# tsunrise/r1cs-spartan

Hardware: AMD Instinct MI355X
Metric: R1CS constraints proved/sec at 2^20 (higher is better)
Workload: dtype bls12-381 Fr/Fq Montgomery (u32 limbs)

## Files before the change

r1cs-spartan_amd/csrc/curve29.hpp:

```cpp
#pragma once
#include "curve_dev.hpp"
#include "ff29.hpp"

namespace spx {

template <class S>
struct R29;
template <>
struct R29<Fq> {
    using T = F29;
    static DEV void unpack(F29& r, const Fq& s) { f29_unpack(r, s.v); }
    static DEV void pack(Fq& s, const F29& r) { f29_pack(s.v, r); }
};
template <>
struct R29<Fq2> {
    using T = F2_29;
    static DEV void unpack(F2_29& r, const Fq2& s) {
        f29_unpack(r.c0, s.c0.v);
        f29_unpack(r.c1, s.c1.v);
    }
    static DEV void pack(Fq2& s, const F2_29& r) {
        f29_pack(s.c0.v, r.c0);
        f29_pack(s.c1.v, r.c1);
    }
// ... 80 lines not shown
template <class F>
DEV void x29_dbl(X29<F>& p) {
    using O = Ops29<F>;
    if (x29_is_inf(p)) return;
    F U, V, W, S, X2, M, t, s2;
    O::add(U, p.y, p.y);
    O::sqr(V, U);
    O::mul(W, U, V);
    O::mul(S, p.x, V);
    O::sqr(X2, p.x);
    O::add(M, X2, X2);
    O::add(M, M, X2);
    O::sqr(t, M);
    O::add(s2, S, S);
    F x3;
    O::template sub<4>(x3, t, s2);
    O::template reduce<8>(x3);
    O::template sub<2>(t, S, x3);
    if constexpr (O::kFusedSum) {
        O::zero(s2);
        O::template sub<2>(s2, s2, W);
        O::mul_sum(p.y, M, t, s2, p.y);
    } else {
        O::mul(t, M, t);
        O::mul(s2, W, p.y);
        O::template sub<2>(p.y, t, s2);
        O::template reduce<4>(p.y);
    }
    p.x = x3;
    O::mul(p.zz, V, p.zz);
    O::mul(p.zzz, W, p.zzz);
}

template <class F>
DEV void x29_madd(X29<F>& p, const F& ax, const F& ay_in, bool neg) {
    using O = Ops29<F>;
    F ay = ay_in;
    if (neg) {
        F z;
        O::zero(z);
        O::template sub<2>(ay, z, ay_in);
    }
    if (x29_is_inf(p)) {
        p.x = ax;
        p.y = ay;
        O::one(p.zz);
        O::one(p.zzz);
        return;
    }
    F U2, S2, P, R;
    O::mul_x2(U2, ax, p.zz, S2, ay, p.zzz);
    O::template sub<8>(P, U2, p.x);
    O::template sub<4>(R, S2, p.y);
    if (O::template zero_lt<16>(P)) {
        if (O::template zero_lt<8>(R))
            x29_from_aff_dbl(p, ax, ay);
        else
            x29_set_inf(p);
        return;
    }
    F PP, PPP, Q, t, w;
    O::template sqr_x2<16, 8>(PP, P, t, R);
    O::mul_x2(PPP, P, PP, Q, p.x, PP);
    O::template sub<2>(w, t, PPP);
    O::add(t, Q, Q);
    O::template sub<4>(w, w, t);
    O::template sub<8>(t, Q, w);
    O::zero(S2);
    O::template sub<4>(S2, S2, p.y);
    O::mul_sum(p.y, t, R, S2, PPP);
    p.x = w;
    O::mul_x2(p.zz, p.zz, PP, p.zzz, p.zzz, PPP);
}

template <class F>
DEV void x29_add(X29<F>& p, const X29<F>& q) {
    using O = Ops29<F>;
    if (x29_is_inf(q)) return;
    if (x29_is_inf(p)) {
        p = q;
        return;
    }
    F U1, U2, S1, S2, P, R;
    O::mul(U1, p.x, q.zz);
    O::mul(U2, q.x, p.zz);
    O::mul(S1, p.y, q.zzz);
    O::mul(S2, q.y, p.zzz);
    O::template sub<2>(P, U2, U1);
    O::template sub<2>(R, S2, S1);
    if (O::template zero_lt<4>(P)) {
        if (O::template zero_lt<4>(R))
            x29_dbl(p);
        else
            x29_set_inf(p);
        return;
    }
    F PP, PPP, Q, t, w;
    O::sqr(PP, P);
    O::mul(PPP, P, PP);
    O::mul(Q, U1, PP);
    O::sqr(t, R);
    O::template sub<2>(w, t, PPP);
    O::add(t, Q, Q);
    O::template sub<4>(w, w, t);
    O::template reduce<8>(w);
// ... 36 lines not shown
```

r1cs-spartan_amd/csrc/msm_common.hip:

```cpp
#include "msm_common.hpp"

#include <algorithm>
#include <cmath>
#include <cstring>
#include <cstdlib>

namespace spx {

__device__ __constant__ constexpr uint32_t kFqR2[12] = {0x1c341746u, 0xf4df1f34u, 0x09d104f1u, 0x0a76e6a6u,
                                                       0x4c95b6d5u, 0x8de5476cu, 0x939d83c0u, 0x67eb88a9u,
                                                       0xb519952du, 0x9a793e85u, 0x92cae3aau, 0x11988fe5u};

struct Digits {
    uint32_t s[8];
    uint32_t carry = 0;
    DEV int32_t next(uint32_t c) {
        const uint32_t full = 1u << c, half = full >> 1;
        uint32_t v = (s[0] & (full - 1)) + carry;
#pragma unroll
        for (int k = 0; k < 7; ++k) s[k] = (s[k] >> c) | (s[k + 1] << (32 - c));
        s[7] >>= c;
        carry = v > half;
        return carry ? (int32_t)v - (int32_t)full : (int32_t)v;
    }
// ... 46 lines not shown
#pragma unroll
    for (int k = 0; k < 8; ++k) d.s[k] = sc.v[k];
    if (I.c == 16 && I.W == 16) {
#pragma unroll
        for (uint32_t w = 0; w < 16; ++w) {
            const int32_t dg = d.at16(w);
            k16.key[w] = digit_key(I, dg);
            k16.ref[w] = digit_ref(I, w, j, dg);
        }
        return true;
    }
    const uint32_t flip = I.c == kMsmWideBits ? d.fold_half() : 0u;
    if (I.c == kMsmWideBits && I.W == kMsmWideWindows) {
#pragma unroll
        for (uint32_t w = 0; w < kMsmWideWindows; ++w) {
            const int32_t dg = d.at17(w);
            k16.key[w] = digit_key(I, dg);
            k16.ref[w] = digit_ref(I, w, j, dg) ^ flip;
        }
        k16.key[15] = ~0u;
        k16.ref[15] = 0u;
        return true;
    }
    for (uint32_t w = 0; w < I.W; ++w) {
        const int32_t dg = d.next(I.c);
        const uint32_t key = digit_key(I, dg);
        if (key != ~0u) f(key, digit_ref(I, w, j, dg) ^ flip);
    }
    return false;
}

static constexpr int kTileThreads = 1024;
static constexpr int kRowThreads = 1024;
static constexpr int kScanThreads = 256;
static constexpr int kBinThreads = 1024;
static constexpr uint32_t kMaxBins = 2048;
static constexpr uint32_t kStagePairs = (uint32_t)kTileThreads * 16;
static constexpr uint32_t kBinStage = 36864;
static constexpr int kMaxLev = 8;
static_assert(((uint64_t)kMaxBins << 8) == kMsmMaxBuckets, "kMsmMaxBuckets (kernels.hpp): kMaxBins bins of 2^8 buckets");
typedef __attribute__((address_space(1))) unsigned int gu32;

struct SortGeom {
    uint32_t nb, sb, nbin;
    uint32_t spt, ntile;
    uint32_t sub;
    uint64_t tot_sc;
};

template <int NT>
DEV uint32_t block_excl_scan(uint32_t v, uint32_t& agg, uint32_t* sh) {
    const int lane = threadIdx.x & 63, w = threadIdx.x >> 6;
    uint32_t x = v;
#pragma unroll
    for (int d = 1; d < 64; d <<= 1) {
        const uint32_t y = __shfl_up(x, d, 64);
        if (lane >= d) x += y;
    }
    if (lane == 63) sh[w] = x;
    __syncthreads();
    uint32_t pre = 0;
    agg = 0;
#pragma unroll
    for (int k = 0; k < NT / 64; ++k) {
        const uint32_t t = sh[k];
        pre += k < w ? t : 0u;
// ... 188 lines not shown
            const uint32_t q = lds_inc(pos, key >> g.sb);
            sref[q] = ref;
            sfine[q] = (uint8_t)(key & fmask);
        };
        if (scalar_keys(insts, prefix, nact, scalars, gi, kk, put)) {
            uint32_t q[16];
#pragma unroll
            for (int w = 0; w < 16; ++w) {
                q[w] = 0u;
                if (kk.key[w] != ~0u) q[w] = lds_inc(pos, kk.key[w] >> g.sb);
            }
#pragma unroll
            for (int w = 0; w < 16; ++w)
                if (kk.key[w] != ~0u) {
                    sref[q[w]] = kk.ref[w];
                    sfine[q[w]] = (uint8_t)(kk.key[w] & fmask);
                }
        }
    }
}

template <int NT, uint32_t STAGE>
struct BinLds {
    uint32_t out[STAGE ? STAGE : 1];
    uint32_t h[256], sh[NT / 64];
};
struct LevPtrs {
    uint32_t* p[kMaxLev + 1];
};
template <int NT, uint32_t STAGE>
__global__ __launch_bounds__(NT) void k_sort_bins(SortGeom g, const uint32_t* __restrict__ binbase,
                                                            uint32_t* __restrict__ st, const uint32_t* __restrict__ sref,
                                                            const uint8_t* __restrict__ sfine, uint32_t* __restrict__ offs,
                                                            uint32_t* __restrict__ refs, uint32_t seg1, int nlev, LevPtrs lev,
                                                            uint32_t* __restrict__ binsum, uint32_t* __restrict__ binpfx,
                                                            uint32_t* __restrict__ ticket, uint32_t* __restrict__ hot,
                                                            uint32_t hot_cap) {
    __shared__ BinLds<NT, STAGE> L;
    __shared__ bool last;
    const uint32_t bin = blockIdx.x, f = threadIdx.x;
    const uint32_t b0 = bin << g.sb, nbk = min(1u << g.sb, g.nb - b0);
    const bool over = (st[0] & kMsmOverflow) != 0;
    const uint32_t base = binbase[bin], n = over ? 0u : binbase[bin + 1] - base;
    const uint32_t a0 = base & ~3u, head = base - a0, nq = n ? (head + n + 3) / 4 : 0u;
    if (f < 256) L.h[f] = 0;
    __syncthreads();
    for (uint32_t q = f; q < nq; q += NT) {
        const uint32_t w4 = *(const uint32_t*)(sfine + a0 + 4 * q);
#pragma unroll
        for (uint32_t e = 0; e < 4; ++e)
            if (4 * q + e - head < n) lds_inc(L.h, (w4 >> (8 * e)) & 0xFFu);
    }
    __syncthreads();
    const uint32_t c = f < nbk ? L.h[f] : 0u;
    uint32_t agg;
    const uint32_t lo = block_excl_scan<NT>(c, agg, L.sh);
    const uint32_t o = base + lo;
    if (f < nbk) offs[b0 + f] = over ? 0u : o;
    uint32_t v = c ? (o + c - 1) / seg1 - o / seg1 + 1 : 0u;
    for (int l = 0; l <= nlev; ++l) {
        if (l) v = (v + kSeg - 1) / kSeg;
        const uint32_t e = block_excl_scan<NT>(v, agg, L.sh);
        if (f < nbk) lev.p[l][b0 + f] = e;
        if (f == 0) st_agent(binsum + (size_t)l * (g.nbin + 1) + bin, agg);
    }
    if (v > kSeg) {
        const uint32_t i = atomicAdd(&st[kMsmStHot], 1u);
        if (i < hot_cap) hot[i] = b0 + f;
    }
    const bool staged = n <= STAGE;
    if (f < 256) L.h[f] = staged ? lo : o;
    __syncthreads();
    for (uint32_t q = f; q < nq; q += NT) {
        const uint32_t w4 = *(const uint32_t*)(sfine + a0 + 4 * q);
        const uint4 r4 = *(const uint4*)(sref + a0 + 4 * q);
        const uint32_t rr[4] = {r4.x, r4.y, r4.z, r4.w};
#pragma unroll
        for (uint32_t e = 0; e < 4; ++e)
            if (4 * q + e - head < n) {
                const uint32_t slot = lds_inc(L.h, (w4 >> (8 * e)) & 0xFFu);
                if (staged)
                    L.out[slot] = rr[e];
                else
                    refs[slot] = rr[e];
            }
    }
    if (staged) {
        __syncthreads();
        for (uint32_t i = f; i < n; i += NT) refs[base + i] = L.out[i];
    }
    if (!handoff_last(ticket, g.nbin, &last)) return;
    for (int l = 0; l <= nlev; ++l) {
        uint32_t carry = 0;
        const uint32_t* src = binsum + (size_t)l * (g.nbin + 1);
        uint32_t* dst = binpfx + (size_t)l * (g.nbin + 1);
        for (uint32_t b = 0; b < g.nbin; b += NT) {
            const uint32_t i = b + f;
            const uint32_t x = i < g.nbin ? ld_agent(src + i) : 0u;
            const uint32_t e = block_excl_scan<NT>(x, agg, L.sh);
            if (i < g.nbin) dst[i] = carry + e;
            carry += agg;
        }
        if (f == 0) dst[g.nbin] = carry;
    }
    if (f == 0) *ticket = 0u;
}

__global__ __launch_bounds__(kScanThreads) void k_sort_final(SortGeom g, int nlev, LevPtrs lev, const uint32_t* __restrict__ binpfx) {
    const uint64_t t = blockIdx.x * (uint64_t)kScanThreads + threadIdx.x;
    const uint32_t l = (uint32_t)(t / (g.nb + 1)), b = (uint32_t)(t % (g.nb + 1));
    if ((int)l > nlev) return;
    const uint32_t* pf = binpfx + (size_t)l * (g.nbin + 1);
    lev.p[l][b] = b < g.nb ? lev.p[l][b] + pf[b >> g.sb] : pf[g.nbin];
}

uint32_t seg1_len(bool) { return kSeg1Default; }

uint32_t seg1_fit(uint32_t seg1, uint64_t refs, int waves_per_simd, int lanes_per_elem) {
    static const int cus = [] {
        int dev = 0, n = 0;
        if (hipGetDevice(&dev) != hipSuccess || hipDeviceGetAttribute(&n, hipDeviceAttributeMultiprocessorCount, dev) != hipSuccess)
            n = 0;
        return n;
    }();
    if (cus <= 0 || refs == 0) return seg1;
    const uint64_t slots = (uint64_t)cus * 4 * waves_per_simd * 64 / lanes_per_elem;
    const uint64_t nthr = (refs + seg1 - 1) / seg1;
    const uint64_t rounds = (nthr + slots - 1) / slots;
    if (rounds > 16) return seg1;
    const uint64_t fit = (refs + rounds * slots - 1) / (rounds * slots);
    return (uint32_t)std::min<uint64_t>(seg1, std::max<uint64_t>(fit, std::min<uint32_t>(seg1, 8)));
}
// ... 12 lines not shown
}
void msm_ws_set_hot(MsmWorkspace* ws, bool on) {
    if (ws) ws->hot_on = on;
}
bool msm_hot_default() {
    static const bool v = [] {
        const char* e = getenv("SPX_MSM_HOT");
        return !(e && atoi(e) == 0 && *e);
    }();
    return v;
}
uint32_t msm_hot_cap(uint64_t tot_refs, uint32_t seg1, int nlev) {
    uint64_t per = 1;
    for (int l = 0; l <= nlev; ++l) per *= kSeg;
    const uint64_t cap = tot_refs / ((per - 1) * std::max<uint32_t>(seg1, 1)) + 1;
    if (cap < tot_refs / (per * std::max<uint32_t>(seg1, 1)) + 1) throw std::runtime_error("MSM: hot-bucket list capacity");
    return (uint32_t)std::min<uint64_t>(cap, 0xffffffffu);
}

static double msm_cap_env() {
    const char* e = getenv("SPX_MSM_CAP_SCALE");
    const double v = e ? atof(e) : 1.0;
    return v > 0 ? v : 1.0;
}

MsmPlan msm_plan(const MsmInst* ih, int ninst, const MsmShard& sh, double cap_scale) {
    MsmPlan o;
    const int G = std::max(1, sh.world);
    int g = 0;
    while ((1 << g) < G) ++g;
    if ((1 << g) != G || sh.rank < 0 || sh.rank >= G) throw std::runtime_error("MSM shard: bad rank / world");
    o.compact = G > 1 && !sh.dense;
    uint64_t tot_refs = 0;
    double split_refs = 0, whole_refs = 0;
    int nsplit = 0;
    for (int i = 0; i < ninst; ++i) {
        MsmInst I = ih[i];
        if (!I.size) continue;
        if (I.c < 3 || I.c > 24) throw std::runtime_error("MSM window bits out of range");
        if (I.W < msm_windows(I.c)) throw std::runtime_error("MSM: too few windows for the window bits");
        const uint32_t lbf = I.c - 1;
        if (G > 1 && (int)lbf - g >= 2) {
            I.lb = lbf - g;
            I.lg = (uint32_t)g;
            I.sel = (uint32_t)sh.rank;
            split_refs += (double)I.size * I.W / G;
            ++nsplit;
        } else if (i % G == sh.rank) {
            I.lb = lbf;
            I.lg = 0;
            I.sel = 0;
            whole_refs += (double)I.size * I.W;
        } else {
            continue;
        }
        I.out = (uint32_t)i;
        I.bucket_off = o.nb;
        I.ref_off = (uint32_t)tot_refs;
        o.nb += 1u << I.lb;
        o.prefix.push_back(o.tot_sc);
        o.tot_sc += I.size;
        tot_refs += (uint64_t)I.size * I.W;
        o.mu_max = std::max(o.mu_max, (double)I.size * I.W / (double)(1u << lbf));
        o.any_split |= I.lg != 0;
        o.insts.push_back(I);
    }
    const int nact = (int)o.insts.size();
    o.prefix.push_back(o.tot_sc);
    if (tot_refs >= 0xffffffffull) throw std::runtime_error("MSM batch too large");
    if (o.compact) {
        const double cap = whole_refs + (split_refs + 8.0 * std::sqrt(split_refs) + 2048.0 * nsplit) * cap_scale * msm_cap_env();
        tot_refs = std::min<uint64_t>(tot_refs, (uint64_t)std::ceil(cap));
    }
    o.tot_refs = tot_refs;
    o.node_off.resize(nact);
    o.cnt.resize(nact);
    uint32_t tot_nodes = 0;
    for (int i = 0; i < nact; ++i) {
        o.node_off[i] = tot_nodes;
        const int lg = (int)o.insts[i].lb - (int)std::min<uint32_t>(kTreeChunkLog, o.insts[i].lb - 1);
        o.cnt[i] = 1u << lg;
        tot_nodes += o.cnt[i];
        o.levels = std::max(o.levels, lg);
    }
    o.wp.assign((size_t)(o.levels + 1) * (nact + 1), 0);
    o.cin.assign((size_t)(o.levels + 1) * nact, 0);
    uint32_t maxc = 1;
    for (int i = 0; i < nact; ++i) maxc = std::max(maxc, o.cnt[i]);
    o.top_from = o.levels + 1;
    for (int lv = 0; lv <= o.levels; ++lv) {
        uint64_t acc = 0;
        for (int i = 0; i < nact; ++i) {
            uint32_t nin = lv == 0 ? (o.cnt[i] * 2) : std::max(1u, o.cnt[i] >> (lv - 1));
            uint32_t nout = lv == 0 ? o.cnt[i] : std::max(1u, o.cnt[i] >> lv);
            o.cin[(size_t)lv * nact + i] = nin;
            o.wp[(size_t)lv * (nact + 1) + i] = acc;
            acc += nout;
        }
        o.wp[(size_t)lv * (nact + 1) + nact] = acc;
        if (lv >= 1 && o.top_from > o.levels && std::max(1u, maxc >> (lv - 1)) <= kTopNodes) o.top_from = lv;
    }
    return o;
}

void msm_upload_plan(MsmWorkspace* ws, MsmPlan& p, hipStream_t s) {
    const int nact = (int)p.insts.size();
    auto al = [](size_t x) { return (x + 15) & ~(size_t)15; };
// ... 38 lines not shown
        while (sb > 0 && (double)(1u << sb) * std::max(p.mu_max, 1.0) > 0.8 * kBinStage) --sb;
    else
        sb = std::min(8, std::max(0, lnb - 9));
    while (sb < 8 && ((uint64_t)p.nb + (1u << sb) - 1) >> sb > kMaxBins) ++sb;
    g.sb = (uint32_t)sb;
    g.nbin = (p.nb + (1u << g.sb) - 1) >> g.sb;
    if (g.nbin > kMaxBins) throw std::runtime_error("MSM batch: too many buckets for the sort");
    const int threads = staged ? kTileThreads : kDirectThreads, tiles_log = staged ? 8 : 9;
    const uint64_t tile_sc = (uint64_t)threads << tiles_log;
    g.spt = (uint32_t)std::min<uint64_t>(64, std::max<uint64_t>(1, (p.tot_sc + tile_sc - 1) / tile_sc));
    const uint64_t ts = (uint64_t)threads * g.spt;
    const uint64_t nt = (p.tot_sc + ts - 1) / ts;
    if (nt > 0x7fffffffull / kSub) throw std::runtime_error("MSM batch: too many tiles");
    g.ntile = (uint32_t)std::max<uint64_t>(1, nt);
    g.sub = staged ? kSub : 1;
    return g;
}

MsmSorted msm_sort(MsmWorkspace* ws, const MsmPlan& p, const Fr* scalars, void* out_dev, size_t out_bytes, hipStream_t s,
                   uint32_t seg1, int nlev) {
    if (nlev > kMaxLev) throw std::runtime_error("MSM: too many partial levels");
    if (out_bytes % 4) throw std::runtime_error("MSM: output bytes not a multiple of 4");
    MsmSorted o;
    bool staged = false;
    const SortGeom g = sort_geom(p, staged);
    const uint32_t nb = p.nb;
    const uint64_t cap = std::max<uint64_t>(p.tot_refs, 1);
    uint32_t* st = (uint32_t*)((uint8_t*)out_dev + out_bytes - 16);
    o.offs = (uint32_t*)ws->offs.ensure(4 * (size_t)(nb + 1));
    o.refs = (uint32_t*)ws->refs.ensure(4 * cap);
    uint32_t* cnt = (uint32_t*)ws->cnt.ensure(4 * (size_t)g.nbin * g.ntile * g.sub);
    uint32_t* bintot = (uint32_t*)ws->bintot.ensure(4 * (size_t)g.nbin);
    uint32_t* binbase = (uint32_t*)ws->binbase.ensure(4 * (size_t)(g.nbin + 1));
    uint32_t* binsum = (uint32_t*)ws->binsum.ensure(4 * 2 * (size_t)(kMaxLev + 1) * (g.nbin + 1));
    uint32_t* binpfx = binsum + (size_t)(kMaxLev + 1) * (g.nbin + 1);
    uint32_t* sref = (uint32_t*)ws->stage_ref.ensure(4 * cap + 16);
    uint8_t* sfine = (uint8_t*)ws->stage_fine.ensure(cap + 16);
    uint32_t* lv = (uint32_t*)ws->lvl.ensure(4 * (size_t)(nb + 1) * (nlev + 1));
    uint32_t* tk = (uint32_t*)ws->tickets.ensure(kTicketBytes);
    if (!ws->tickets_zeroed) {
        HIPCHK(hipMemsetAsync(tk, 0, kTicketBytes, s));
        ws->tickets_zeroed = true;
    }
    LevPtrs lp{};
    for (int l = 0; l <= nlev; ++l) lp.p[l] = lv + (size_t)l * (nb + 1);
    o.hot_cap = msm_hot_cap(p.tot_refs, seg1, nlev);
    o.hot = (uint32_t*)ws->hot.ensure(4 * (size_t)o.hot_cap);
    const int nact = (int)p.insts.size();
    kp_begin(KP_SORT, s);
    hipLaunchKernelGGL(k_sort_count, dim3(g.ntile * g.sub), dim3(kCountThreads), 0, s, p.d_insts, p.d_prefix, nact, scalars, g,
                       cnt, (uint32_t*)out_dev, (uint32_t)(out_bytes / 4));
    const uint32_t cap32 = (uint32_t)std::min<uint64_t>(cap, 0xffffffffu);
    if (staged) {
        hipLaunchKernelGGL(k_sort_scan<kRowThreads>, dim3(g.nbin), dim3(kRowThreads), 0, s, cnt, g, bintot, binbase, tk, cap32,
                           st, o.offs + nb);
        hipLaunchKernelGGL(k_sort_scatter, dim3(g.ntile), dim3(kTileThreads), 0, s, p.d_insts, p.d_prefix, nact, scalars, g, cnt,
                           binbase, st, sref, sfine);
        hipLaunchKernelGGL((k_sort_bins<kBinThreads, kBinStage>), dim3(g.nbin), dim3(kBinThreads), 0, s, g, binbase, st, sref,
                           sfine, o.offs, o.refs, seg1, nlev, lp, binsum, binpfx, tk + 16, o.hot, o.hot_cap);
    } else {
        hipLaunchKernelGGL(k_sort_scan<kDirectThreads>, dim3(g.nbin), dim3(kDirectThreads), 0, s, cnt, g, bintot, binbase, tk,
                           cap32, st, o.offs + nb);
        hipLaunchKernelGGL(k_sort_scatter_direct, dim3(g.ntile), dim3(kDirectThreads), 0, s, p.d_insts, p.d_prefix, nact, scalars,
                           g, cnt, binbase, st, sref, sfine);
        hipLaunchKernelGGL((k_sort_bins<kDirectThreads, 0>), dim3(g.nbin), dim3(kDirectThreads), 0, s, g, binbase, st, sref,
                           sfine, o.offs, o.refs, seg1, nlev, lp, binsum, binpfx, tk + 16, o.hot, o.hot_cap);
    }
    const uint64_t nfin = (uint64_t)(nlev + 1) * (nb + 1);
    hipLaunchKernelGGL(k_sort_final, dim3((unsigned)((nfin + kScanThreads - 1) / kScanThreads)), dim3(kScanThreads), 0, s, g,
                       nlev, lp, binpfx);
    kp_end(64.0 * p.tot_sc + 14.0 * p.tot_refs + 16.0 * g.nbin * g.ntile * g.sub, s, (double)p.tot_refs);
    o.np_off = lp.p[0];
    for (int l = 1; l <= nlev; ++l) o.lev.push_back(lp.p[l]);
    return o;
}

DEV bool fq_canon_to_mont(Fq& r, const Fq& c) {
    uint32_t br = 0;
#pragma unroll
    for (int i = 0; i < 12; ++i) {
        uint64_t d = (uint64_t)c.v[i] - kFqP[i] - br;
        br = (uint32_t)(d >> 63);
    }
    Fq r2;
#pragma unroll
    for (int i = 0; i < 12; ++i) r2.v[i] = kFqR2[i];
    fe_mul(r, c, r2);
    return br != 0;
}

template <int NF>
__global__ void k_points_from_bytes(Fq* pts, uint64_t n, int* err) {
    for (uint64_t j = blockIdx.x * (uint64_t)blockDim.x + threadIdx.x; j < n; j += (uint64_t)gridDim.x * blockDim.x) {
        Fq* p = pts + j * NF;
        Fq last;
        load_vec(last, p + NF - 1);
        const uint32_t flags = last.v[11] >> 30;
        bool ok = true;
        if (flags & 1u) {
            Fq z;
// ... 72 lines not shown
```

r1cs-spartan_amd/csrc/msm_common.hpp:

```cpp
#pragma once
#include <algorithm>
#include <cstring>
#include <stdexcept>
#include <string>
#include <vector>

#include "kernels.hpp"

namespace spx {

static constexpr uint32_t kSeg1Default = 64;
uint32_t seg1_len(bool g2);
uint32_t seg1_fit(uint32_t seg1, uint64_t refs, int waves_per_simd, int lanes_per_elem);
static constexpr uint32_t kSeg = 4;
static constexpr uint32_t kTreeChunkLog = 2;
static constexpr uint32_t kTopNodes = 32;
static constexpr int kLight = 256;
static constexpr int kHeavy = 64;

#define HIPCHK(x)                                                                                     \
    do {                                                                                              \
        hipError_t e_ = (x);                                                                          \
        if (e_ != hipSuccess) throw std::runtime_error(std::string("HIP error: ") + hipGetErrorString(e_) + \
                                                       " at " __FILE__ ":" + std::to_string(__LINE__)); \
    } while (0)

template <class F>
DEV bool aff_is_sentinel(const Aff<F>& a) {
    return FieldOps<F>::is_zero(a.x) && FieldOps<F>::is_zero(a.y);
}
template <class F>
DEV void aff_set_sentinel(Aff<F>& a) {
    FieldOps<F>::zero(a.x);
    FieldOps<F>::zero(a.y);
}

DEV int find_slot(const uint64_t* prefix, int n, uint64_t g) {
    int lo = 0, hi = n - 1;
    while (lo < hi) {
        int mid = (lo + hi + 1) >> 1;
        if (prefix[mid] <= g)
            lo = mid;
        else
            hi = mid - 1;
    }
    return lo;
// ... 35 lines not shown
    PinArena() { HIPCHK(hipHostMalloc((void**)&p, kCap)); }
    ~PinArena() {
        if (p) (void)hipHostFree(p);
    }
    template <class T>
    T* stage(const T* src, size_t count) {
        const size_t o = (used + 255) & ~(size_t)255, b = sizeof(T) * count;
        if (o + b > kCap) throw std::runtime_error("MSM pinned staging arena exhausted");
        used = o + b;
        memcpy(p + o, src, b);
        return (T*)(p + o);
    }
    void reset() { used = 0; }
};

struct MsmWorkspace {
    DBuf tables, offs, refs, pa, pb, tree_a, tree_b;
    DBuf cnt, bintot, binbase, binsum, stage_ref, stage_fine, lvl, tickets;
    bool tickets_zeroed = false;
    DBuf hot;
    bool hot_on = true;
    double cap_scale = 1.0;
    PinArena pin;
};

struct MsmPlan {
    std::vector<MsmInst> insts;
    std::vector<uint64_t> prefix;
    uint32_t nb = 0;
    uint64_t tot_sc = 0;
    uint64_t tot_refs = 0;
    bool compact = false;
    double mu_max = 0;
    bool any_split = false;
    std::vector<uint32_t> node_off, cnt;
    int levels = 0;
    int top_from = 1;
    std::vector<uint64_t> wp;
    std::vector<uint32_t> cin;
    MsmInst* d_insts = nullptr;
    uint64_t *d_prefix = nullptr, *d_wp = nullptr;
    uint32_t *d_cin = nullptr, *d_noff = nullptr;
};
MsmPlan msm_plan(const MsmInst* ih, int ninst, const MsmShard& sh, double cap_scale);
void msm_upload_plan(MsmWorkspace* ws, MsmPlan& p, hipStream_t s);

uint32_t msm_hot_cap(uint64_t tot_refs, uint32_t seg1, int nlev);
struct MsmSorted {
    uint32_t *offs, *refs, *np_off;
    std::vector<uint32_t*> lev;
    uint32_t* hot = nullptr;
    uint32_t hot_cap = 0;
};
MsmSorted msm_sort(MsmWorkspace* ws, const MsmPlan& p, const Fr* scalars, void* out_dev, size_t out_bytes, hipStream_t s,
                   uint32_t seg1, int nlev);

}
```

r1cs-spartan_amd/csrc/msm_impl.hpp:

```cpp
#pragma once
#include "curve29.hpp"
#include "fq2pair.hpp"
#include "msm_common.hpp"

namespace spx {

template <class F>
struct Acc;
struct AffRaw {
    Fq x, y;
};
template <>
struct Acc<Fq> {
    using Pt = G1Slot;
    using T = F29;
    using TA = F29;
    static constexpr int kLanes = 1, kWaves = 1;
    static DEV void ld_raw(AffRaw& a, const G1Slot* p) { load_vec(*(Aff<Fq>*)&a, &p->p); }
    static DEV void unpack(T& x, T& y, const AffRaw& a) {
        f29_unpack(x, a.x.v);
        f29_unpack(y, a.y.v);
    }
    static DEV void ld_aff(T& x, T& y, const G1Slot* p) {
        AffRaw a;
// ... 160 lines not shown
}

template <class F>
struct TreeLanes {
    static constexpr int v = 2 * Acc<F>::kLanes;
};
template <class F>
DEV void tree_add(X29<typename Acc<F>::T>& p, const X29<typename Acc<F>::T>& q) {
    x29_add_split(p, q);
}
template <class F>
DEV void tree_dbl(X29<typename Acc<F>::T>& p) {
    x29_dbl_split(p);
}
template <class F>
DEV uint64_t tree_elem() {
    return (blockIdx.x * (uint64_t)blockDim.x + threadIdx.x) / TreeLanes<F>::v;
}
template <class F>
static unsigned tree_blocks(uint64_t elems) {
    return (unsigned)((elems * TreeLanes<F>::v + kHeavy - 1) / kHeavy);
}

template <class F>
DEV uint64_t acc_elem() {
    return (blockIdx.x * (uint64_t)blockDim.x + threadIdx.x) / Acc<F>::kLanes;
}
template <class F>
static unsigned acc_blocks(uint64_t elems) {
    return (unsigned)((elems * Acc<F>::kLanes + kHeavy - 1) / kHeavy);
}

template <class F>
__global__ __launch_bounds__(kHeavy, Acc<F>::kWaves) void k_accum_aff(const uint32_t* __restrict__ off, uint32_t nb,
                                                                      const uint32_t* __restrict__ pfx,
                                                                      const uint32_t* __restrict__ refs,
                                                                      const typename Acc<F>::Pt* __restrict__ pts,
                                                                      Xyzz<F>* __restrict__ out, uint32_t seg1) {
    using A = Acc<F>;
    using T = typename A::TA;
    const uint32_t t = (uint32_t)acc_elem<F>();
    const uint32_t total = off[nb];
    uint32_t e = t * seg1;
    if (e >= total) return;
    const uint32_t end = min(e + seg1, total);
    uint32_t b = find_bucket(off, nb, e);
    uint32_t bend = off[b + 1];
    uint32_t slot = pfx[b] + (t - off[b] / seg1);
    X29<T> acc;
    x29_set_inf(acc);
    for (; e < end; ++e) {
        if (e == bend) {
            A::st(out + slot, acc);
            x29_set_inf(acc);
            do {
                ++b;
            } while (off[b + 1] <= e);
            bend = off[b + 1];
            slot = pfx[b];
        }
        const uint32_t r = refs[e];
        T px, py;
        A::ld_aff(px, py, pts + (r & 0x7fffffffu));
        if (A::aff_sentinel(px, py)) continue;
        x29_madd(acc, px, py, (r >> 31) != 0);
    }
    A::st(out + slot, acc);
}

template <class F>
__global__ __launch_bounds__(kHeavy, Acc<F>::kWaves) void k_accum_xyzz(const uint32_t* __restrict__ segoff, uint32_t nb,
                                                                       const uint32_t* __restrict__ off,
                                                                       const Xyzz<F>* __restrict__ in,
                                                                       Xyzz<F>* __restrict__ out) {
    using A = Acc<F>;
    using T = typename A::T;
    const uint32_t s = (uint32_t)tree_elem<F>();
    if (s >= segoff[nb]) return;
    const uint32_t b = find_bucket(segoff, nb, s);
    const uint32_t k = s - segoff[b];
    const uint32_t start = off[b] + k * kSeg;
    const uint32_t end = min(start + kSeg, off[b + 1]);
    X29<T> acc;
    A::ld(acc, in + start);
    for (uint32_t e = start + 1; e < end; ++e) {
        X29<T> p;
        A::ld(p, in + e);
        tree_add<F>(acc, p);
    }
    A::st(out + s, acc);
}

static constexpr int kHotThreads = 256;
static constexpr uint32_t kHotGrid = 64;
template <class F>
__global__ __launch_bounds__(kHotThreads, 1) void k_accum_hot(const uint32_t* __restrict__ hot, uint32_t cap,
                                                              uint32_t* __restrict__ st, const uint32_t* __restrict__ off,
                                                              Xyzz<F>* P) {
    using A = Acc<F>;
    using T = typename A::T;
// ... 220 lines not shown
}

static int msm_levels_env() {
    static const int v = [] {
        const char* e = getenv("SPX_MSM_LEVELS");
        return e ? atoi(e) : -1;
    }();
    return v;
}
static int msm_seg1_env() {
    static const int v = [] {
        const char* e = getenv("SPX_MSM_SEG1");
        return e ? atoi(e) : 0;
    }();
    return v;
}

template <class F>
static void msm_run_t(MsmWorkspace* ws, const MsmInst* ih, int ninst, const typename Acc<F>::Pt* pts, const Fr* scalars,
                      void* out_dev, hipStream_t s, const MsmShard& sh) {
    if (ninst <= 0) return;
    const bool g2 = sizeof(F) == sizeof(Fq2);
    const size_t psz = sizeof(Xyzz<F>);
    const size_t ob = msm_out_bytes(g2, ninst);
    MsmPlan pl = msm_plan(ih, ninst, sh, ws->cap_scale);
    const int nact = (int)pl.insts.size();
    if (!nact) {
        HIPCHK(hipMemsetAsync(out_dev, 0, ob, s));
        return;
    }
    msm_upload_plan(ws, pl, s);
    const uint32_t nb = pl.nb;
    const uint64_t tot_refs = pl.tot_refs;
    uint32_t kSeg1 = seg1_fit(seg1_len(g2), tot_refs, Acc<F>::kWaves, Acc<F>::kLanes);
    if (msm_seg1_env() > 0) kSeg1 = std::min<uint32_t>(kSeg1, (uint32_t)msm_seg1_env());
    const double mu = pl.mu_max;
    int nlev = 0;
    for (uint32_t m = (uint32_t)std::ceil((mu + 6.0 * std::sqrt(mu) + 16.0) / kSeg1) + 1; m > 1; m = (m + kSeg - 1) / kSeg)
        ++nlev;
    if (msm_levels_env() >= 0) nlev = std::min(nlev, msm_levels_env());
    MsmSorted so = msm_sort(ws, pl, scalars, out_dev, ob, s, kSeg1, nlev);
    const uint64_t max_segs = tot_refs / kSeg1 + nb + 1;
    auto* PA = (Xyzz<F>*)ws->pa.ensure(psz * max_segs);
    auto* PB = (Xyzz<F>*)ws->pb.ensure(psz * (max_segs / kSeg + nb + 1));
    uint32_t* cur_off = so.np_off;
    uint32_t* nxt_off = nullptr;
    const uint64_t nthr = (tot_refs + kSeg1 - 1) / kSeg1;
    kp_begin(g2 ? KP_ACC_G2 : KP_ACC_G1, s);
    hipLaunchKernelGGL(k_accum_aff<F>, dim3(acc_blocks<F>(nthr)), dim3(kHeavy), 0, s, so.offs, nb, cur_off, so.refs, pts, PA,
                       kSeg1);
    kp_end((double)tot_refs * (4.0 + sizeof(Aff<F>)) + (double)(tot_refs / kSeg1) * psz, s, (double)tot_refs);
    Xyzz<F>* cur = PA;
    Xyzz<F>* nxt = PB;
    uint64_t cur_max_segs = max_segs;
    for (int l = 0; l < nlev; ++l) {
        nxt_off = so.lev[l];
        uint64_t nsegs = cur_max_segs / kSeg + nb + 1;
        kp_begin(g2 ? KP_ACCX_G2 : KP_ACCX_G1, s);
        hipLaunchKernelGGL(k_accum_xyzz<F>, dim3(tree_blocks<F>(nsegs)), dim3(kHeavy), 0, s, nxt_off, nb, cur_off, cur, nxt);
        kp_end((double)(cur_max_segs + nsegs) * psz, s, (double)cur_max_segs);
        std::swap(cur, nxt);
        std::swap(cur_off, nxt_off);
        cur_max_segs = nsegs;
    }
    uint32_t* stw = (uint32_t*)((uint8_t*)out_dev + ob - 16);
    if (ws->hot_on) {
        kp_begin(g2 ? KP_ACCX_G2 : KP_ACCX_G1, s);
        hipLaunchKernelGGL(k_accum_hot<F>, dim3(std::min(so.hot_cap, kHotGrid)), dim3(kHotThreads), 0, s, so.hot, so.hot_cap,
                           stw, cur_off, cur);
        kp_end(0.0, s);
    }
    uint32_t tot_nodes = 0;
    for (int i = 0; i < nact; ++i) tot_nodes += pl.cnt[i];
    auto* TA = (Xyzz<F>*)ws->tree_a.ensure(3 * psz * std::max<uint32_t>(tot_nodes, 1));
    auto* TB = (Xyzz<F>*)ws->tree_b.ensure(3 * psz * std::max<uint32_t>(tot_nodes, 1));
    Xyzz<F>* A3[3] = {TA, TA + tot_nodes, TA + 2 * (size_t)tot_nodes};
    Xyzz<F>* B3[3] = {TB, TB + tot_nodes, TB + 2 * (size_t)tot_nodes};
    kp_begin(g2 ? KP_RED_G2 : KP_RED_G1, s);
    {
        uint64_t work = pl.wp[nact];
        hipLaunchKernelGGL(k_tree_chunk<F>, dim3(tree_blocks<F>(work)), dim3(kHeavy), 0, s, pl.d_insts, pl.d_wp, nact,
                           pl.d_noff, cur_off, cur, A3[0], A3[1], A3[2], ws->hot_on ? 1u : 0u, stw);
    }
    for (int lv = 1; lv < pl.top_from; ++lv) {
        uint64_t work = 3 * pl.wp[(size_t)lv * (nact + 1) + nact];
        hipLaunchKernelGGL(k_tree_level<F>, dim3(tree_blocks<F>(work)), dim3(kHeavy), 0, s,
                           pl.d_wp + (size_t)lv * (nact + 1), nact, pl.d_noff, pl.d_cin + (size_t)lv * nact, A3[0], A3[1],
                           A3[2], B3[0], B3[1], B3[2]);
        std::swap(A3, B3);
    }
// ... 149 lines not shown
```

Before: 66.09 million.

## Split bucket accumulation by additions instead of refs to balance MSM work

The first-level bucket accumulation is now partitioned by the number of point additions rather than the number of references. The first point of each bucket counts as a free load, so each thread handles a fixed count of real madds. A new k_sort_levels kernel computes per-bucket addition offsets and the level prefix sums that used to live in k_sort_bins. The madd loop is restructured so empty-accumulator loads skip the infinity branch, and the seg1 fit uses an expected-adds estimate. This adds an extra kernel launch and more complex walk logic, with some risk of divergence or off-by-one issues at bucket boundaries.

```diff
diff --git a/r1cs-spartan_amd/csrc/accum_split.hpp b/r1cs-spartan_amd/csrc/accum_split.hpp
--- /dev/null
+++ b/r1cs-spartan_amd/csrc/accum_split.hpp
@@ -0,0 +1,74 @@
+#pragma once
+#include <cstdint>
+
+#if defined(__HIPCC__) || defined(__CUDACC__)
+#define SPX_HD __host__ __device__ inline
+#else
+#define SPX_HD inline
+#endif
+
+namespace spx {
+namespace asplit {
+
+SPX_HD uint64_t elems(uint64_t adds, uint32_t seg1) { return adds / seg1 + 1; }
+
+SPX_HD uint32_t first_elem(uint32_t a, uint32_t seg1) { return a / seg1; }
+
+SPX_HD uint32_t part_count(uint32_t a, uint32_t c, uint32_t seg1) { return c ? (a + c - 1) / seg1 - a / seg1 + 1 : 0u; }
+
+SPX_HD uint64_t max_partials(uint64_t refs, uint32_t nb, uint32_t seg1) { return refs / seg1 + nb + 1; }
+SPX_HD uint64_t max_segments(uint64_t prev, uint32_t nb, uint32_t kseg) { return prev / kseg + nb + 1; }
+
+struct Walk {
+    uint32_t e, b, bbeg, bend, rem, total, slot;
+
+    SPX_HD bool begin(const uint32_t* off, const uint32_t* aoff, const uint32_t* pfx, uint32_t nb, uint32_t seg1, uint32_t t) {
+        total = off[nb];
+        if (!total) return false;
+        if (t == 0) {
+            e = 0;
+            b = 0;
+            while (off[b + 1] == 0) ++b;
+            rem = seg1 - 1;
+            slot = pfx[b];
+        } else {
+            const uint64_t K64 = (uint64_t)t * seg1;
+            if (K64 > aoff[nb]) return false;
+            const uint32_t K = (uint32_t)K64;
+            uint32_t lo = 0, hi = nb;
+            while (lo < hi) {
+                const uint32_t mid = (lo + hi + 1) >> 1;
+                if (aoff[mid] < K)
+                    lo = mid;
+                else
+                    hi = mid - 1;
+            }
+            if (lo == nb) return false;
+            b = lo;
+            const uint32_t a = aoff[b];
+            e = off[b] + (K - a);
+            rem = seg1;
+            slot = pfx[b] + (t - first_elem(a, seg1));
+        }
+        bbeg = off[b];
+        bend = off[b + 1];
+        return true;
+    }
+    SPX_HD bool more() const { return e != total && (rem != 0 || e == bend || e == bbeg); }
+    SPX_HD bool at_boundary() const { return e == bend; }
+    SPX_HD void next_bucket(const uint32_t* off, const uint32_t* pfx) {
+        do {
+            ++b;
+        } while (off[b + 1] <= e);
+        bbeg = e;
+        bend = off[b + 1];
+        slot = pfx[b];
+    }
+    SPX_HD uint32_t take() {
+        rem -= (e != bbeg) ? 1u : 0u;
+        return e++;
+    }
+};
+
+}
+}
diff --git a/r1cs-spartan_amd/csrc/curve29.hpp b/r1cs-spartan_amd/csrc/curve29.hpp
--- a/r1cs-spartan_amd/csrc/curve29.hpp
+++ b/r1cs-spartan_amd/csrc/curve29.hpp
@@ -136,22 +136,28 @@
     O::mul(p.zzz, W, p.zzz);
 }
 
-template <class F>
-DEV void x29_madd(X29<F>& p, const F& ax, const F& ay_in, bool neg) {
-    using O = Ops29<F>;
-    F ay = ay_in;
+
+template <class F>
+DEV void x29_aff_sign(F& ay, const F& ay_in, bool neg) {
+    using O = Ops29<F>;
+    ay = ay_in;
     if (neg) {
         F z;
         O::zero(z);
         O::template sub<2>(ay, z, ay_in);
     }
-    if (x29_is_inf(p)) {
-        p.x = ax;
-        p.y = ay;
-        O::one(p.zz);
-        O::one(p.zzz);
-        return;
-    }
+}
+template <class F>
+DEV void x29_from_aff(X29<F>& p, const F& ax, const F& ay) {
+    using O = Ops29<F>;
+    p.x = ax;
+    p.y = ay;
+    O::one(p.zz);
+    O::one(p.zzz);
+}
+template <class F>
+DEV void x29_madd_ne(X29<F>& p, const F& ax, const F& ay) {
+    using O = Ops29<F>;
     F U2, S2, P, R;
     O::mul_x2(U2, ax, p.zz, S2, ay, p.zzz);
     O::template sub<8>(P, U2, p.x);
@@ -175,6 +181,16 @@
     O::mul_sum(p.y, t, R, S2, PPP);
     p.x = w;
     O::mul_x2(p.zz, p.zz, PP, p.zzz, p.zzz, PPP);
+}
+template <class F>
+DEV void x29_madd(X29<F>& p, const F& ax, const F& ay_in, bool neg) {
+    F ay;
+    x29_aff_sign(ay, ay_in, neg);
+    if (x29_is_inf(p)) {
+        x29_from_aff(p, ax, ay);
+        return;
+    }
+    x29_madd_ne(p, ax, ay);
 }
 
 template <class F>
diff --git a/r1cs-spartan_amd/csrc/msm_common.hip b/r1cs-spartan_amd/csrc/msm_common.hip
--- a/r1cs-spartan_amd/csrc/msm_common.hip
+++ b/r1cs-spartan_amd/csrc/msm_common.hip
@@ -102,6 +102,7 @@
 
 static constexpr int kTileThreads = 1024;
 static constexpr int kRowThreads = 1024;
+static constexpr int kLevThreads = 256;
 static constexpr int kScanThreads = 256;
 static constexpr int kBinThreads = 1024;
 static constexpr uint32_t kMaxBins = 2048;
@@ -356,12 +357,9 @@
 __global__ __launch_bounds__(NT) void k_sort_bins(SortGeom g, const uint32_t* __restrict__ binbase,
                                                             uint32_t* __restrict__ st, const uint32_t* __restrict__ sref,
                                                             const uint8_t* __restrict__ sfine, uint32_t* __restrict__ offs,
-                                                            uint32_t* __restrict__ refs, uint32_t seg1, int nlev, LevPtrs lev,
-                                                            uint32_t* __restrict__ binsum, uint32_t* __restrict__ binpfx,
-                                                            uint32_t* __restrict__ ticket, uint32_t* __restrict__ hot,
-                                                            uint32_t hot_cap) {
+                                                            uint32_t* __restrict__ refs, uint32_t* __restrict__ aoff,
+                                                            uint32_t* __restrict__ nzsum) {
     __shared__ BinLds<NT, STAGE> L;
-    __shared__ bool last;
     const uint32_t bin = blockIdx.x, f = threadIdx.x;
     const uint32_t b0 = bin << g.sb, nbk = min(1u << g.sb, g.nb - b0);
     const bool over = (st[0] & kMsmOverflow) != 0;
@@ -381,17 +379,9 @@
     const uint32_t lo = block_excl_scan<NT>(c, agg, L.sh);
     const uint32_t o = base + lo;
     if (f < nbk) offs[b0 + f] = over ? 0u : o;
-    uint32_t v = c ? (o + c - 1) / seg1 - o / seg1 + 1 : 0u;
-    for (int l = 0; l <= nlev; ++l) {
-        if (l) v = (v + kSeg - 1) / kSeg;
-        const uint32_t e = block_excl_scan<NT>(v, agg, L.sh);
-        if (f < nbk) lev.p[l][b0 + f] = e;
-        if (f == 0) st_agent(binsum + (size_t)l * (g.nbin + 1) + bin, agg);
-    }
-    if (v > kSeg) {
-        const uint32_t i = atomicAdd(&st[kMsmStHot], 1u);
-        if (i < hot_cap) hot[i] = b0 + f;
-    }
+    const uint32_t zin = block_excl_scan<NT>(c ? 1u : 0u, agg, L.sh);
+    if (f < nbk) aoff[b0 + f] = over ? 0u : o - zin;
+    if (f == 0) nzsum[bin] = agg;
     const bool staged = n <= STAGE;
     if (f < 256) L.h[f] = staged ? lo : o;
     __syncthreads();
@@ -413,6 +403,42 @@
         __syncthreads();
         for (uint32_t i = f; i < n; i += NT) refs[base + i] = L.out[i];
     }
+}
+
+__global__ __launch_bounds__(kLevThreads) void k_sort_levels(SortGeom g, uint32_t* __restrict__ st,
+                                                             const uint32_t* __restrict__ offs, uint32_t* __restrict__ aoff,
+                                                             const uint32_t* __restrict__ nzsum, uint32_t seg1, int nlev,
+                                                             LevPtrs lev, uint32_t* __restrict__ binsum,
+                                                             uint32_t* __restrict__ binpfx, uint32_t* __restrict__ ticket,
+                                                             uint32_t* __restrict__ hot, uint32_t hot_cap) {
+    constexpr int NT = kLevThreads;
+    __shared__ uint32_t sh[NT / 64];
+    __shared__ bool last;
+    const uint32_t bin = blockIdx.x, f = threadIdx.x;
+    const uint32_t b0 = bin << g.sb, nbk = min(1u << g.sb, g.nb - b0);
+    uint32_t agg, nz = 0;
+    for (uint32_t i = f; i < (bin ? bin : g.nbin); i += NT) nz += nzsum[i];
+    (void)block_excl_scan<NT>(nz, agg, sh);
+    const uint32_t zb = bin ? agg : 0u;
+    if (bin == 0 && f == 0) aoff[g.nb] = offs[g.nb] - agg;
+    uint32_t a = 0, c = 0;
+    if (f < nbk) {
+        const uint32_t o = offs[b0 + f];
+        c = offs[b0 + f + 1] - o;
+        a = aoff[b0 + f] - zb;
+        aoff[b0 + f] = a;
+    }
+    uint32_t v = asplit::part_count(a, c, seg1);
+    for (int l = 0; l <= nlev; ++l) {
+        if (l) v = (v + kSeg - 1) / kSeg;
+        const uint32_t e = block_excl_scan<NT>(v, agg, sh);
+        if (f < nbk) lev.p[l][b0 + f] = e;
+        if (f == 0) st_agent(binsum + (size_t)l * (g.nbin + 1) + bin, agg);
+    }
+    if (v > kSeg) {
+        const uint32_t i = atomicAdd(&st[kMsmStHot], 1u);
+        if (i < hot_cap) hot[i] = b0 + f;
+    }
     if (!handoff_last(ticket, g.nbin, &last)) return;
     for (int l = 0; l <= nlev; ++l) {
         uint32_t carry = 0;
@@ -421,7 +447,7 @@
         for (uint32_t b = 0; b < g.nbin; b += NT) {
             const uint32_t i = b + f;
             const uint32_t x = i < g.nbin ? ld_agent(src + i) : 0u;
-            const uint32_t e = block_excl_scan<NT>(x, agg, L.sh);
+            const uint32_t e = block_excl_scan<NT>(x, agg, sh);
             if (i < g.nbin) dst[i] = carry + e;
             carry += agg;
         }
@@ -500,7 +526,7 @@
     if ((1 << g) != G || sh.rank < 0 || sh.rank >= G) throw std::runtime_error("MSM shard: bad rank / world");
     o.compact = G > 1 && !sh.dense;
     uint64_t tot_refs = 0;
-    double split_refs = 0, whole_refs = 0;
+    double split_refs = 0, whole_refs = 0, exp_nz = 0;
     int nsplit = 0;
     for (int i = 0; i < ninst; ++i) {
         MsmInst I = ih[i];
@@ -530,6 +556,8 @@
         o.tot_sc += I.size;
         tot_refs += (uint64_t)I.size * I.W;
         o.mu_max = std::max(o.mu_max, (double)I.size * I.W / (double)(1u << lbf));
+        const double mu_i = (double)I.size * I.W / (double)(1u << lbf);
+        exp_nz += (double)(1u << I.lb) * (1.0 - std::exp(-mu_i));
         o.any_split |= I.lg != 0;
         o.insts.push_back(I);
     }
@@ -541,6 +569,7 @@
         tot_refs = std::min<uint64_t>(tot_refs, (uint64_t)std::ceil(cap));
     }
     o.tot_refs = tot_refs;
+    o.exp_adds = (uint64_t)std::max(1.0, (double)tot_refs - std::min(exp_nz, (double)tot_refs));
     o.node_off.resize(nact);
     o.cnt.resize(nact);
     uint32_t tot_nodes = 0;
@@ -645,11 +674,13 @@
     uint32_t* cnt = (uint32_t*)ws->cnt.ensure(4 * (size_t)g.nbin * g.ntile * g.sub);
     uint32_t* bintot = (uint32_t*)ws->bintot.ensure(4 * (size_t)g.nbin);
     uint32_t* binbase = (uint32_t*)ws->binbase.ensure(4 * (size_t)(g.nbin + 1));
-    uint32_t* binsum = (uint32_t*)ws->binsum.ensure(4 * 2 * (size_t)(kMaxLev + 1) * (g.nbin + 1));
+    uint32_t* binsum = (uint32_t*)ws->binsum.ensure(4 * (2 * (size_t)(kMaxLev + 1) + 1) * (g.nbin + 1));
     uint32_t* binpfx = binsum + (size_t)(kMaxLev + 1) * (g.nbin + 1);
+    uint32_t* nzsum = binpfx + (size_t)(kMaxLev + 1) * (g.nbin + 1);
     uint32_t* sref = (uint32_t*)ws->stage_ref.ensure(4 * cap + 16);
     uint8_t* sfine = (uint8_t*)ws->stage_fine.ensure(cap + 16);
-    uint32_t* lv = (uint32_t*)ws->lvl.ensure(4 * (size_t)(nb + 1) * (nlev + 1));
+    uint32_t* lv = (uint32_t*)ws->lvl.ensure(4 * (size_t)(nb + 1) * (nlev + 2));
+    o.aoff = lv + (size_t)(nlev + 1) * (nb + 1);
     uint32_t* tk = (uint32_t*)ws->tickets.ensure(kTicketBytes);
     if (!ws->tickets_zeroed) {
         HIPCHK(hipMemsetAsync(tk, 0, kTicketBytes, s));
@@ -670,15 +701,17 @@
         hipLaunchKernelGGL(k_sort_scatter, dim3(g.ntile), dim3(kTileThreads), 0, s, p.d_insts, p.d_prefix, nact, scalars, g, cnt,
                            binbase, st, sref, sfine);
         hipLaunchKernelGGL((k_sort_bins<kBinThreads, kBinStage>), dim3(g.nbin), dim3(kBinThreads), 0, s, g, binbase, st, sref,
-                           sfine, o.offs, o.refs, seg1, nlev, lp, binsum, binpfx, tk + 16, o.hot, o.hot_cap);
+                           sfine, o.offs, o.refs, o.aoff, nzsum);
     } else {
         hipLaunchKernelGGL(k_sort_scan<kDirectThreads>, dim3(g.nbin), dim3(kDirectThreads), 0, s, cnt, g, bintot, binbase, tk,
                            cap32, st, o.offs + nb);
         hipLaunchKernelGGL(k_sort_scatter_direct, dim3(g.ntile), dim3(kDirectThreads), 0, s, p.d_insts, p.d_prefix, nact, scalars,
                            g, cnt, binbase, st, sref, sfine);
         hipLaunchKernelGGL((k_sort_bins<kDirectThreads, 0>), dim3(g.nbin), dim3(kDirectThreads), 0, s, g, binbase, st, sref,
-                           sfine, o.offs, o.refs, seg1, nlev, lp, binsum, binpfx, tk + 16, o.hot, o.hot_cap);
-    }
+                           sfine, o.offs, o.refs, o.aoff, nzsum);
+    }
+    hipLaunchKernelGGL(k_sort_levels, dim3(g.nbin), dim3(kLevThreads), 0, s, g, st, o.offs, o.aoff, nzsum, seg1, nlev, lp, binsum,
+                       binpfx, tk + 16, o.hot, o.hot_cap);
     const uint64_t nfin = (uint64_t)(nlev + 1) * (nb + 1);
     hipLaunchKernelGGL(k_sort_final, dim3((unsigned)((nfin + kScanThreads - 1) / kScanThreads)), dim3(kScanThreads), 0, s, g,
                        nlev, lp, binpfx);
diff --git a/r1cs-spartan_amd/csrc/msm_common.hpp b/r1cs-spartan_amd/csrc/msm_common.hpp
--- a/r1cs-spartan_amd/csrc/msm_common.hpp
+++ b/r1cs-spartan_amd/csrc/msm_common.hpp
@@ -5,13 +5,14 @@
 #include <string>
 #include <vector>
 
+#include "accum_split.hpp"
 #include "kernels.hpp"
 
 namespace spx {
 
 static constexpr uint32_t kSeg1Default = 64;
 uint32_t seg1_len(bool g2);
-uint32_t seg1_fit(uint32_t seg1, uint64_t refs, int waves_per_simd, int lanes_per_elem);
+uint32_t seg1_fit(uint32_t seg1, uint64_t adds, int waves_per_simd, int lanes_per_elem);
 static constexpr uint32_t kSeg = 4;
 static constexpr uint32_t kTreeChunkLog = 2;
 static constexpr uint32_t kTopNodes = 32;
@@ -113,6 +114,7 @@
     uint64_t tot_refs = 0;
     bool compact = false;
     double mu_max = 0;
+    uint64_t exp_adds = 0;
     bool any_split = false;
     std::vector<uint32_t> node_off, cnt;
     int levels = 0;
@@ -128,7 +130,7 @@
 
 uint32_t msm_hot_cap(uint64_t tot_refs, uint32_t seg1, int nlev);
 struct MsmSorted {
-    uint32_t *offs, *refs, *np_off;
+    uint32_t *offs, *refs, *aoff, *np_off;
     std::vector<uint32_t*> lev;
     uint32_t* hot = nullptr;
     uint32_t hot_cap = 0;
diff --git a/r1cs-spartan_amd/csrc/msm_impl.hpp b/r1cs-spartan_amd/csrc/msm_impl.hpp
--- a/r1cs-spartan_amd/csrc/msm_impl.hpp
+++ b/r1cs-spartan_amd/csrc/msm_impl.hpp
@@ -216,40 +216,46 @@
 }
 
 template <class F>
-__global__ __launch_bounds__(kHeavy, Acc<F>::kWaves) void k_accum_aff(const uint32_t* __restrict__ off, uint32_t nb,
+__global__ __launch_bounds__(kHeavy, Acc<F>::kWaves) void k_accum_aff(const uint32_t* __restrict__ off,
+                                                                      const uint32_t* __restrict__ aoff, uint32_t nb,
                                                                       const uint32_t* __restrict__ pfx,
                                                                       const uint32_t* __restrict__ refs,
                                                                       const typename Acc<F>::Pt* __restrict__ pts,
                                                                       Xyzz<F>* __restrict__ out, uint32_t seg1) {
     using A = Acc<F>;
     using T = typename A::TA;
-    const uint32_t t = (uint32_t)acc_elem<F>();
-    const uint32_t total = off[nb];
-    uint32_t e = t * seg1;
-    if (e >= total) return;
-    const uint32_t end = min(e + seg1, total);
-    uint32_t b = find_bucket(off, nb, e);
-    uint32_t bend = off[b + 1];
-    uint32_t slot = pfx[b] + (t - off[b] / seg1);
+    asplit::Walk w;
+    if (!w.begin(off, aoff, pfx, nb, seg1, (uint32_t)acc_elem<F>())) return;
     X29<T> acc;
     x29_set_inf(acc);
-    for (; e < end; ++e) {
-        if (e == bend) {
-            A::st(out + slot, acc);
-            x29_set_inf(acc);
-            do {
-                ++b;
-            } while (off[b + 1] <= e);
-            bend = off[b + 1];
-            slot = pfx[b];
-        }
-        const uint32_t r = refs[e];
+    uint32_t rn = refs[w.e];
+    for (;;) {
         T px, py;
-        A::ld_aff(px, py, pts + (r & 0x7fffffffu));
-        if (A::aff_sentinel(px, py)) continue;
-        x29_madd(acc, px, py, (r >> 31) != 0);
-    }
-    A::st(out + slot, acc);
+        bool add = false;
+        while (w.more()) {
+            if (w.at_boundary()) {
+                A::st(out + w.slot, acc);
+                x29_set_inf(acc);
+                w.next_bucket(off, pfx);
+            }
+            const bool empty = x29_is_inf(acc);
+            const uint32_t r = rn;
+            w.take();
+            if (w.e != w.total) rn = refs[w.e];
+            T ly;
+            A::ld_aff(px, ly, pts + (r & 0x7fffffffu));
+            if (A::aff_sentinel(px, ly)) continue;
+            x29_aff_sign(py, ly, (r >> 31) != 0);
+            if (!empty) {
+                add = true;
+                break;
+            }
+            x29_from_aff(acc, px, py);
+        }
+        if (!add) break;
+        x29_madd_ne(acc, px, py);
+    }
+    A::st(out + w.slot, acc);
 }
 
 template <class F>
@@ -536,30 +542,30 @@
     msm_upload_plan(ws, pl, s);
     const uint32_t nb = pl.nb;
     const uint64_t tot_refs = pl.tot_refs;
-    uint32_t kSeg1 = seg1_fit(seg1_len(g2), tot_refs, Acc<F>::kWaves, Acc<F>::kLanes);
+    uint32_t kSeg1 = seg1_fit(seg1_len(g2), pl.exp_adds, Acc<F>::kWaves, Acc<F>::kLanes);
     if (msm_seg1_env() > 0) kSeg1 = std::min<uint32_t>(kSeg1, (uint32_t)msm_seg1_env());
     const double mu = pl.mu_max;
     int nlev = 0;
-    for (uint32_t m = (uint32_t)std::ceil((mu + 6.0 * std::sqrt(mu) + 16.0) / kSeg1) + 1; m > 1; m = (m + kSeg - 1) / kSeg)
+    for (uint32_t m = (uint32_t)std::ceil((mu + 6.0 * std::sqrt(mu) + 15.0) / kSeg1) + 1; m > 1; m = (m + kSeg - 1) / kSeg)
         ++nlev;
     if (msm_levels_env() >= 0) nlev = std::min(nlev, msm_levels_env());
     MsmSorted so = msm_sort(ws, pl, scalars, out_dev, ob, s, kSeg1, nlev);
-    const uint64_t max_segs = tot_refs / kSeg1 + nb + 1;
+    const uint64_t max_segs = asplit::max_partials(tot_refs, nb, kSeg1);
     auto* PA = (Xyzz<F>*)ws->pa.ensure(psz * max_segs);
-    auto* PB = (Xyzz<F>*)ws->pb.ensure(psz * (max_segs / kSeg + nb + 1));
+    auto* PB = (Xyzz<F>*)ws->pb.ensure(psz * asplit::max_segments(max_segs, nb, kSeg));
     uint32_t* cur_off = so.np_off;
     uint32_t* nxt_off = nullptr;
-    const uint64_t nthr = (tot_refs + kSeg1 - 1) / kSeg1;
+    const uint64_t nthr = asplit::elems(tot_refs, kSeg1);
     kp_begin(g2 ? KP_ACC_G2 : KP_ACC_G1, s);
-    hipLaunchKernelGGL(k_accum_aff<F>, dim3(acc_blocks<F>(nthr)), dim3(kHeavy), 0, s, so.offs, nb, cur_off, so.refs, pts, PA,
-                       kSeg1);
+    hipLaunchKernelGGL(k_accum_aff<F>, dim3(acc_blocks<F>(nthr)), dim3(kHeavy), 0, s, so.offs, so.aoff, nb, cur_off, so.refs,
+                       pts, PA, kSeg1);
     kp_end((double)tot_refs * (4.0 + sizeof(Aff<F>)) + (double)(tot_refs / kSeg1) * psz, s, (double)tot_refs);
     Xyzz<F>* cur = PA;
     Xyzz<F>* nxt = PB;
     uint64_t cur_max_segs = max_segs;
     for (int l = 0; l < nlev; ++l) {
         nxt_off = so.lev[l];
-        uint64_t nsegs = cur_max_segs / kSeg + nb + 1;
+        uint64_t nsegs = asplit::max_segments(cur_max_segs, nb, kSeg);
         kp_begin(g2 ? KP_ACCX_G2 : KP_ACCX_G1, s);
         hipLaunchKernelGGL(k_accum_xyzz<F>, dim3(tree_blocks<F>(nsegs)), dim3(kHeavy), 0, s, nxt_off, nb, cur_off, cur, nxt);
         kp_end((double)(cur_max_segs + nsegs) * psz, s, (double)cur_max_segs);
```

Measured after the change: 66.25 million, median of 2. No clear change (+0.2%).
